# cgisky1980/Qwen3-TTS-Rust

Measured on AMD Instinct MI355X. Metric: audio_sec_per_s, higher is better.
Workload: dtype bf16

## Files before the change

qwen3-tts-rust_amd/csrc/q3_engine.h:

```cpp
#pragma once
#include <algorithm>
#include <cstddef>
#include <atomic>
#include <mutex>
#include <string>
#include <vector>

#include "../../include/q3tts.h"
#include "q3_kernels.h"

static_assert(sizeof(q3tts_request) == 80 && offsetof(q3tts_request, text_stream) == 12 && offsetof(q3tts_request, prompt) == 16 &&
              offsetof(q3tts_request, text_open) == 44 && offsetof(q3tts_request, seed) == 48 && offsetof(q3tts_request, prefix) == 72, "q3tts_request layout");

struct Q3Voc;
struct Q3Mel;
struct Q3Clone;

struct Q3Tfm {
    int L = 0, d = 0, Hq = 0, Hkv = 0, hd = 0, F = 0, nq = 0, nkv = 0, nqkv = 0, head_n = 0;
    std::vector<float*> attn_norm, ffn_norm, qn, kn;
    std::vector<uint4*> wqkv, wo, wgu, wd;
    float* out_norm = nullptr;
    uint4* head = nullptr;
    std::vector<uint16_t*> sqkv, so, sgu, sd; uint16_t* shead = nullptr; bool q8 = false;
// ... 49 lines not shown
    std::vector<float*> codec;
    const float** codec_dev = nullptr;
    std::vector<float*> pproj;
    float* proj_w = nullptr;
    float* proj_b = nullptr;
    float* qkv0 = nullptr;
    float* tts_pad = nullptr;
    float* marker_row = nullptr;
    int B = 0;
    std::vector<int> buckets; int cur_bucket = -1;
    std::vector<std::atomic<long long>> bucket_steps;
    std::atomic<long long> kvp_launches{0}, kvp_group_max{0};
    std::vector<int> row_of_slot, slot_of_row;
    Q3Slot* slots = nullptr;
    Q3Slot* slots_host = nullptr;
    int* codes = nullptr;
    float* rng = nullptr;
    Q3Lane lane;
    Q3Scratch sc_pre;
    Q3Rows pf;
    int *pf_pos = nullptr, *pf_slot = nullptr;
    int* pf_seg = nullptr;
    Q3PromptRow* prow_dev = nullptr; int prow_cap = 0;
    float* spk_dev = nullptr; int* refcodes_dev = nullptr;
    float temperature = 0.7f; int top_k = 40; float top_p = 0.9f; int has_seed = 0; uint64_t seed = 0;
    int max_steps = 512;
    float p_temperature = 0.0f; int p_top_k = 0; float p_top_p = 1.0f; float rep_penalty = 1.0f;
    int pred_force = 0, pred_variant = 0;
    int streams_open = 0;
    int* ts_ids = nullptr; int* ts_cnt = nullptr; int2* ts_cur = nullptr;
    std::vector<char> ts_slot; int ts_variant = 0, ts_used = 0;
    float* prng = nullptr;
    uint32_t* seen = nullptr; int seen_words = 0;
    hipEvent_t ev0 = nullptr, ev1 = nullptr, ev2 = nullptr, ev3 = nullptr;
    std::vector<hipEvent_t> fin_ev;
    q3tts_timings tm{};
    Q3Voc* voc = nullptr;
    Q3Mel* mel = nullptr;
    Q3Clone* clone = nullptr;
    int probe = 0, probe_kind = 0;
    std::vector<hipEvent_t> probe_ev;
    int probe_i = 0;
    double probe_ms = 0, probe_empty_ms = 0; long long probe_cnt = 0, probe_empty_cnt = 0, row_steps = 0;
    int dev_pcm_on = 0; float* dev_pcm = nullptr; int dev_pcm_n = 0; size_t dev_pcm_stride = 0;
    int out_rate = 0; Q3Resamp rs_out{}; std::vector<Q3Resamp> rs_cache;
    float* rs_stage = nullptr; size_t rs_stage_stride = 0, rs_stage_cap = 0;
    double hp_launch = 0, hp_sync = 0;
    float *park_logits = nullptr, *park_x = nullptr;
    float* first_chunk_host = nullptr;
    std::atomic<q3tts_session*> session{nullptr};
    std::mutex err_mu;
};

struct q3tts_prefix {
    q3tts_engine* e = nullptr;
    int P = 0, np = 0;
    uint16_t *k = nullptr, *v = nullptr;
    std::atomic<int> state{1};
    bool released = false; int qrefs = 0;
};
size_t q3_prefix_store_bytes(const q3tts_engine* e, int np);

int q3_set_err(q3tts_engine* e, int code, const std::string& msg);
int q3_refuse_in_session(q3tts_engine* e);
#define Q3_NOT_IN_SESSION(e) do { if ((e) && (e)->session.load()) return q3_refuse_in_session(e); } while (0)
#define Q3_HIP(e, call)                                                                                         \
    do {                                                                                                        \
// ... 52 lines not shown
int q3_launch_gemm(q3tts_engine* e, const Q3Tfm& t, const Q3BGemm& g, hipStream_t s, hipEvent_t* probe = nullptr, int kind = -1);

void q3_rope_tables(int n_pos, int hd, float theta, const int* sections, std::vector<float>& cs, std::vector<float>& sn);

void q3_stdrng_f32(uint64_t seed, int n, float* out);

void q3_mel_destroy(q3tts_engine* e);
int q3_mel_run(q3tts_engine* e, const float* audio, int64_t n_samples, int32_t* n_frames, float** out_dev);
void q3_clone_destroy(q3tts_engine* e);
int q3_voc_create(q3tts_engine* e);
void q3_voc_destroy(q3tts_engine* e);
int q3_voc_reset(q3tts_engine* e, int slot);
int q3_voc_decode(q3tts_engine* e, int slot, int f0, int nf, int is_last, hipStream_t s);
int q3_voc_decode_batch(q3tts_engine* e, const int* slots, const int* real, int ns, int nf, hipStream_t s, int beside_decoder);
void q3_voc_mark_last(q3tts_engine* e, int slot);
float* q3_voc_pcm(q3tts_engine* e, int slot);
int q3_voc_samples(q3tts_engine* e, int slot);
int q3_voc_samples_per_frame(const q3tts_engine* e);
size_t q3_voc_pcm_stride(const q3tts_engine* e);

int q3_resample_get(q3tts_engine* e, int rate_in, int rate_out, Q3Resamp* out);
int q3_resample_slot(q3tts_engine* e, int b, long long first_out, int count, int n_valid, bool is_final, hipStream_t s);

enum { BOS_TOKEN = 151672, EOS_TOKEN = 151673 };

int q3_plan_rows(q3tts_engine* e, const std::vector<int>& live);
int q3_admit_many(q3tts_engine* e, const int* slots, const q3tts_request* const* reqs, int count, int* rc);
struct Q3AdmItem {
    int slot; const q3tts_request* r;
    q3tts_prefix* keep; int keep_rows;
    const q3tts_prompt_desc* voice; const float* embd; int n_tok;
};
int q3_admit_items(q3tts_engine* e, const Q3AdmItem* items, int count, int* rc);
int q3_run_chunk(q3tts_engine* e, int CH);
int q3_clone_audio_encode_run(q3tts_engine* e, const float* audio, int64_t n_samples, int64_t* codes, int32_t cap_frames, int32_t* n_frames);
int q3_clone_speaker_encode_run(q3tts_engine* e, const float* audio, int64_t n_samples, float* spk_emb);
int q3_resample_run(q3tts_engine* e, const float* in, int64_t n_in, int32_t rate_in, int32_t rate_out, float* out, int64_t cap, int64_t* n_out);
int q3_text_rows_set(q3tts_engine* e, int b, const int32_t* T, int from, int n, int n_frames);
int q3_park_rows(q3tts_engine* e, int b, bool save);
void q3_text_trailing(const q3tts_request* r, std::vector<int32_t>& T);
int q3_pred_force_variant(q3tts_engine* e, int force);
int q3_voc_dispatch(q3tts_engine* e, const char* live, const char* want, int* voc_frames, bool more, bool* first);
double q3_now_ms();
```

qwen3-tts-rust_amd/csrc/q3_engine.hip:

```cpp
#include "q3_engine.h"
#include "q3_gguf.h"

#include <chrono>
#include <cmath>
#include <cstdio>
#include <cstdlib>
#include <cstring>

static thread_local std::string g_err;

int q3_set_err(q3tts_engine* e, int code, const std::string& msg) {
    if (e) { std::lock_guard<std::mutex> lk(e->err_mu); e->err = msg; }
    g_err = msg;
    return code;
}
extern "C" const char* q3tts_last_error(const q3tts_engine* e) {
    if (!e) return g_err.c_str();
    if (!e->session.load()) return e->err.c_str();
    static thread_local std::string copy;
    std::lock_guard<std::mutex> lk(const_cast<q3tts_engine*>(e)->err_mu);
    copy = e->err;
    return copy.c_str();
}
int q3_refuse_in_session(q3tts_engine* e) {
// ... 175 lines not shown
                              std::to_string(mm.t_head_dim) + ", ratio " + std::to_string(R) + ", n_ctx = " + std::to_string(cfg->n_ctx));
    }
    int ndev = 0;
    if (hipGetDeviceCount(&ndev) != hipSuccess || ndev <= 0)
        return q3_set_err(nullptr, Q3TTS_ERR_DEVICE, "no HIP device: libq3tts has no CPU fallback");
    if (cfg->device < 0 || cfg->device >= ndev) return q3_set_err(nullptr, Q3TTS_ERR_INVALID, "device ordinal out of range");
    q3tts_engine* e = new q3tts_engine();
    e->cfg = *cfg; e->cfg.weights_path = nullptr;
    e->max_steps = cfg->max_steps_cap < 512 ? cfg->max_steps_cap : 512;
    auto fail = [&](int rc) { std::string m = e->err; q3tts_engine_destroy(e); g_err = m; return rc; };
#define TRYC(x) do { int rc__ = (x); if (rc__ != Q3TTS_OK) return fail(rc__); } while (0)
#define HIPC(call) do { hipError_t er__ = (call); if (er__ != hipSuccess) { q3_set_err(e, Q3TTS_ERR_DEVICE, std::string(#call) + ": " + hipGetErrorString(er__)); return fail(Q3TTS_ERR_DEVICE); } } while (0)
    HIPC(hipSetDevice(cfg->device));
    {
        size_t free_b = 0, total_b = 0;
        HIPC(hipMemGetInfo(&free_b, &total_b));
        const unsigned long long need = engine_footprint(*cfg);
        if (need > (unsigned long long)free_b) {
            q3_set_err(e, Q3TTS_ERR_OOM, "engine needs at least " + std::to_string(need) + " bytes of device memory for max_batch = " + std::to_string(cfg->max_batch) +
                       ", n_ctx = " + std::to_string(cfg->n_ctx) + (cfg->kv_q8_0 ? " (Q8_0 cache)" : "") + "; the device has " + std::to_string((unsigned long long)free_b) +
                       (cfg->kv_q8_0 ? " bytes free (fewer slots or a smaller n_ctx)" : " bytes free (fewer slots, a smaller n_ctx, or kv_q8_0 = 1: the cache in 0.53 of the bytes)"));
            return fail(Q3TTS_ERR_OOM);
        }
    }
    q3_bgemm_prepare();
    if (cfg->talker_q8_0 == 2 || cfg->predictor_q8_0 == 2) q3_bgemm8_prepare();
    HIPC(hipStreamCreateWithFlags(&e->stream, hipStreamNonBlocking));
    if (getenv("Q3TTS_VOC_SERIAL") && atoi(getenv("Q3TTS_VOC_SERIAL"))) e->vstream = e->stream;
    else if (getenv("Q3TTS_VOC_CUMASK")) {
        uint32_t w = (uint32_t)strtoul(getenv("Q3TTS_VOC_CUMASK"), nullptr, 16), mask[8];
        for (auto& x : mask) x = w;
        HIPC(hipExtStreamCreateWithCUMask(&e->vstream, 8, mask));
    } else HIPC(hipStreamCreateWithFlags(&e->vstream, hipStreamNonBlocking));
    HIPC(hipEventCreate(&e->ev0)); HIPC(hipEventCreate(&e->ev1)); HIPC(hipEventCreate(&e->ev2)); HIPC(hipEventCreate(&e->ev3));
    e->fin_ev.resize(cfg->max_batch, nullptr);
    for (auto& ev : e->fin_ev) HIPC(hipEventCreateWithFlags(&ev, hipEventDisableTiming));
    const q3tts_model_config& m = e->cfg.model;
    const int B = cfg->max_batch;
    e->B = B;
    hipStream_t s = e->stream;
    const std::string wdir = cfg->weights_path ? cfg->weights_path : "";
    Q3Gguf gt, gp;
    std::string er;
    if (!wdir.empty() && (gt.open(wdir + "/qwen3_tts_talker.gguf", er) || gp.open(wdir + "/qwen3_tts_predictor.gguf", er))) { q3_set_err(e, Q3TTS_ERR_INVALID, er); return fail(Q3TTS_ERR_INVALID); }
    TRYC(q3_tfm_init(e, e->T, {.grp = Q3G_TALKER, .L = m.t_n_layer, .d = m.t_d_model, .Hq = m.t_n_head, .Hkv = m.t_n_kv_head, .hd = m.t_head_dim, .F = m.t_d_ffn,
                               .head_n = m.t_vocab, .theta = m.t_rope_theta, .sections = m.t_mrope_sections, .n_ctx = cfg->n_ctx, .n_slots = B, .kv8 = cfg->kv_q8_0},
                     wdir.empty() ? nullptr : &gt, "qwen3_tts_talker.gguf", cfg->talker_q8_0));
    TRYC(q3_tfm_init(e, e->P, {.grp = Q3G_PRED, .L = m.p_n_layer, .d = m.p_d_model, .Hq = m.p_n_head, .Hkv = m.p_n_kv_head, .hd = m.p_head_dim, .F = m.p_d_ffn,
                               .head_n = (m.n_codebooks - 1) * m.codebook_size, .theta = m.p_rope_theta, .sections = nullptr, .n_ctx = 64, .n_slots = B, .kv8 = 0},
                     wdir.empty() ? nullptr : &gp, "qwen3_tts_predictor.gguf", cfg->predictor_q8_0));
    TRYC(q3_assets_init(e, wdir));
    TRYC(q3_pred_table_init(e));
    TRYC(q3_dalloc(e, &e->slots, (size_t)B));
    HIPC(hipHostMalloc((void**)&e->slots_host, sizeof(Q3Slot) * 2 * B, hipHostMallocDefault));
    memset(e->slots_host, 0, sizeof(Q3Slot) * 2 * B);
    TRYC(q3_dalloc(e, &e->codes, (size_t)B * cfg->max_steps_cap * m.n_codebooks)); TRYC(q3_dalloc(e, &e->rng, (size_t)B * cfg->max_steps_cap));
    TRYC(q3_dalloc(e, &e->prng, (size_t)B * cfg->max_steps_cap * (m.n_codebooks - 1)));
    e->seen_words = (m.sample_limit + 31) / 32;
    TRYC(q3_dalloc(e, &e->seen, (size_t)B * e->seen_words));
    TRYC(q3_dalloc(e, &e->ts_ids, (size_t)B * cfg->max_steps_cap)); TRYC(q3_dalloc(e, &e->ts_cnt, (size_t)B)); TRYC(q3_dalloc(e, &e->ts_cur, (size_t)B));
    TRYC(q3_dalloc(e, &e->park_logits, (size_t)B * m.t_vocab)); TRYC(q3_dalloc(e, &e->park_x, (size_t)B * m.t_d_model));
    e->ts_slot.assign(B, 0);
    {
        const int nb = B;
        const int nqkv_max = std::max(e->T.nqkv, e->P.nqkv), nq_max = std::max(e->T.nq, e->P.nq), F_max = std::max(e->T.F, e->P.F);
        Q3Lane& L = e->lane;
        L.nb = nb;
// ... 43 lines not shown
    return Q3TTS_OK;
}

extern "C" void q3tts_engine_destroy(q3tts_engine* e) {
    if (!e) return;
    if (q3tts_session* ss = e->session.load()) q3tts_session_close(ss);
    hipSetDevice(e->cfg.device);
    if (e->stream) hipStreamSynchronize(e->stream);
    if (e->vstream) hipStreamSynchronize(e->vstream);
    if (e->voc) q3_voc_destroy(e);
    q3_mel_destroy(e);
    q3_clone_destroy(e);
    if (e->first_chunk_host) hipHostFree(e->first_chunk_host);
    {
        Q3Lane& L = e->lane;
        if (L.stream) hipStreamSynchronize(L.stream);
        for (auto ge : L.execs) if (ge) hipGraphExecDestroy(ge);
        for (auto gr : L.graphs) if (gr) hipGraphDestroy(gr);
        for (auto ge : L.execs_s) if (ge) hipGraphExecDestroy(ge);
        for (auto gr : L.graphs_s) if (gr) hipGraphDestroy(gr);
        for (int v = 0; v < 2; ++v) {
            for (auto ge : L.execs_t[v]) if (ge) hipGraphExecDestroy(ge);
            for (auto gr : L.graphs_t[v]) if (gr) hipGraphDestroy(gr);
        }
        if (L.ev_begin) hipEventDestroy(L.ev_begin); if (L.ev_end) hipEventDestroy(L.ev_end);
        if (L.stream) hipStreamDestroy(L.stream);
    }
    for (void* p : e->allocs) hipFree(p);
    hipFree(e->dev_pcm);
    hipFree(e->rs_stage);
    if (e->slots_host) hipHostFree(e->slots_host);
    for (auto ev : e->fin_ev) if (ev) hipEventDestroy(ev);
    for (auto ev : e->probe_ev) if (ev) hipEventDestroy(ev);
    if (e->ev0) hipEventDestroy(e->ev0); if (e->ev1) hipEventDestroy(e->ev1); if (e->ev2) hipEventDestroy(e->ev2); if (e->ev3) hipEventDestroy(e->ev3);
    if (e->stream) hipStreamDestroy(e->stream);
    if (e->vstream && e->vstream != e->stream) hipStreamDestroy(e->vstream);
    delete e;
}

extern "C" int q3tts_set_sampler(q3tts_engine* e, float temperature, int32_t top_k, float top_p, int32_t has_seed, uint64_t seed) {
    if (!e) return q3_set_err(nullptr, Q3TTS_ERR_INVALID, "null engine");
    Q3_NOT_IN_SESSION(e);
    e->temperature = temperature; e->top_k = top_k; e->top_p = top_p; e->has_seed = has_seed; e->seed = seed;
    return Q3TTS_OK;
}
static int refuse_busy(q3tts_engine* e) {
    if (e->streams_open > 0) return q3_set_err(e, Q3TTS_ERR_STATE, "a stream is open on this engine (q3tts_stream_end first)");
    return Q3TTS_OK;
}
static int set_pred_variant(q3tts_engine* e, int variant) {
    if (variant && e->cfg.model.codebook_size > Q3_SAMP_MAX) return q3_set_err(e, Q3TTS_ERR_INVALID, "the Predictor sampler needs codebook_size <= 4096");
    if (!variant) { e->pred_variant = 0; return Q3TTS_OK; }
    Q3_HIP(e, hipSetDevice(e->cfg.device));
    if (q3_pred_next_prepare() != 0) return q3_set_err(e, Q3TTS_ERR_DEVICE, "the Predictor sampler's kernel: the device refused its LDS size (hipFuncSetAttribute)");
    e->pred_variant = variant;
    Q3Lane& L = e->lane;
    if (!L.execs.empty() && L.execs_s.empty()) {
        Q3_HIP(e, hipStreamSynchronize(e->stream));
        const int rc = q3_capture_frames(e, L.graphs_s, L.execs_s);
        if (rc != Q3TTS_OK) {
            for (auto ge : L.execs_s) if (ge) hipGraphExecDestroy(ge);
            for (auto gr : L.graphs_s) if (gr) hipGraphDestroy(gr);
            L.execs_s.clear(); L.graphs_s.clear(); e->pred_variant = 0;
            return rc;
        }
    }
    return Q3TTS_OK;
// ... 141 lines not shown
    return Q3TTS_OK;
}

static int plan_rows(q3tts_engine* e, const std::vector<int>& live_in) {
    Q3Lane& L = e->lane;
    const int B = e->B;
    std::vector<int> live(live_in);
    std::sort(live.begin(), live.end());
    int bi = 0;
    while (bi + 1 < (int)e->buckets.size() && e->buckets[bi] < (int)live.size()) ++bi;
    bool ok = bi == e->cur_bucket;
    if (ok) for (int b : live) if (e->row_of_slot[b] >= e->buckets[bi]) { ok = false; break; }
    if (ok) return Q3TTS_OK;
    std::vector<int> slot_of_row(B, -1), perm(B), used(B, 0);
    int r = 0;
    for (int b : live) { slot_of_row[r++] = b; used[b] = 1; }
    for (int b = 0; b < B && r < B; ++b) if (!used[b]) slot_of_row[r++] = b;
    for (r = 0; r < B; ++r) perm[r] = e->row_of_slot[slot_of_row[r]];
    hipStream_t s = e->stream;
    Q3_HIP(e, hipMemcpyAsync(L.perm, perm.data(), (size_t)B * 4, hipMemcpyHostToDevice, s));
    Q3_HIP(e, hipMemcpyAsync(L.slot_id, slot_of_row.data(), (size_t)B * 4, hipMemcpyHostToDevice, s));
    q3_launch_gather_rows(L.logits_tmp, L.logits, L.perm, B, e->cfg.model.t_vocab, s);
    Q3_HIP(e, hipMemcpyAsync(L.logits, L.logits_tmp, (size_t)B * e->cfg.model.t_vocab * 4, hipMemcpyDeviceToDevice, s));
    q3_launch_gather_rows(L.logits_tmp, L.T.x, L.perm, B, e->cfg.model.t_d_model, s);
    Q3_HIP(e, hipMemcpyAsync(L.T.x, L.logits_tmp, (size_t)B * e->cfg.model.t_d_model * 4, hipMemcpyDeviceToDevice, s));
    Q3_HIP(e, hipStreamSynchronize(s));
    for (r = 0; r < B; ++r) e->row_of_slot[slot_of_row[r]] = r;
    e->slot_of_row = slot_of_row;
    e->cur_bucket = bi;
    return Q3TTS_OK;
}

static double now_ms();
static int run_chunk(q3tts_engine* e, int CH, float* dev_ms) {
    hipStream_t s = e->stream;
    Q3Lane& L = e->lane;
    const double hp0 = now_ms();
    Q3_HIP(e, hipEventRecord(e->ev1, s));
    Q3_HIP(e, hipStreamWaitEvent(L.stream, e->ev1, 0));
    Q3_HIP(e, hipEventRecord(L.ev_begin, L.stream));
    e->probe_i = 0;
    if (e->probe) { hipEventRecord(e->probe_ev[8], L.stream); hipEventRecord(e->probe_ev[9], L.stream); }
    bool ts = false;
    for (char f : e->ts_slot) ts |= f != 0;
    e->ts_variant = ts ? 1 : 0;
    const std::vector<hipGraphExec_t>& execs = ts ? L.execs_t[e->pred_variant ? 1 : 0] : e->pred_variant ? L.execs_s : L.execs;
    for (int i = 0; i < CH; ++i) {
        if (!execs.empty() && !e->probe) { Q3_HIP(e, hipGraphLaunch(execs[e->cur_bucket], L.stream)); }
        else {
            if (q3_record_frame(e, L, L.stream, e->buckets[e->cur_bucket])) return q3_set_err(e, Q3TTS_ERR_INVALID, "frame step: a kernel launch was refused for this model shape");
            Q3_HIP(e, hipGetLastError());
        }
    }
    e->row_steps += (long long)CH * e->buckets[e->cur_bucket];
    e->bucket_steps[e->cur_bucket].fetch_add(CH, std::memory_order_relaxed);
    Q3_HIP(e, hipEventRecord(L.ev_end, L.stream));
    Q3_HIP(e, hipStreamWaitEvent(s, L.ev_end, 0));
    Q3_HIP(e, hipEventRecord(e->ev3, s));
    Q3_HIP(e, hipMemcpyAsync(e->slots_host, e->slots, sizeof(Q3Slot) * e->B, hipMemcpyDeviceToHost, s));
    const double hp1 = now_ms();
    Q3_HIP(e, hipStreamSynchronize(s));
    e->hp_launch += hp1 - hp0; e->hp_sync += now_ms() - hp1;
    if (dev_ms) { *dev_ms = 0.0f; hipEventElapsedTime(dev_ms, L.ev_begin, L.ev_end); }
    for (int i = 0; i + 1 < e->probe_i; i += 2) {
        float ms = 0.0f;
        if (hipEventElapsedTime(&ms, e->probe_ev[i], e->probe_ev[i + 1]) == hipSuccess) { e->probe_ms += ms; ++e->probe_cnt; }
    }
    if (e->probe) {
        float ms = 0.0f;
        if (hipEventElapsedTime(&ms, e->probe_ev[8], e->probe_ev[9]) == hipSuccess) { e->probe_empty_ms += ms; ++e->probe_empty_cnt; }
    }
    return Q3TTS_OK;
}

static uint64_t wall_seed() {
    return (uint64_t)std::chrono::duration_cast<std::chrono::nanoseconds>(std::chrono::system_clock::now().time_since_epoch()).count();
}

struct Adm { int b; const q3tts_request* r; int n, row0, max_steps, P; q3tts_prefix* keep; int keep_rows; };

void q3_text_trailing(const q3tts_request* r, std::vector<int32_t>& T) {
    T.clear();
    const q3tts_prompt_desc* p = r->prompt;
    for (int i = 1; p && i < p->n_text; ++i) T.push_back((int32_t)p->text_ids[i]);
    if (!(r->text_open == 1)) T.push_back(EOS_TOKEN);
}
int q3_text_rows_set(q3tts_engine* e, int b, const int32_t* T, int from, int n, int n_frames) {
    const int cap = e->cfg.max_steps_cap, c = std::min(std::max(n, 0), cap);
    hipStream_t s = e->stream;
    from = std::max(from, 0);
    if (from < c) Q3_HIP(e, hipMemcpyAsync(e->ts_ids + (size_t)b * cap + from, T + from, (size_t)(c - from) * 4, hipMemcpyHostToDevice, s));
    const int2 cur = n_frames >= 0 && n_frames < c ? make_int2(1, T[n_frames]) : make_int2(0, 0);
    Q3_HIP(e, hipMemcpyAsync(e->ts_cnt + b, &c, 4, hipMemcpyHostToDevice, s));
    Q3_HIP(e, hipMemcpyAsync(e->ts_cur + b, &cur, sizeof(cur), hipMemcpyHostToDevice, s));
    Q3_HIP(e, hipStreamSynchronize(s));
    return Q3TTS_OK;
}
int q3_park_rows(q3tts_engine* e, int b, bool save) {
    const q3tts_model_config& m = e->cfg.model;
    Q3Lane& L = e->lane;
    const size_t row = (size_t)e->row_of_slot[b], nl = (size_t)m.t_vocab, nx = (size_t)m.t_d_model;
    float *lg = L.logits + row * nl, *x = L.T.x + row * nx, *plg = e->park_logits + (size_t)b * nl, *px = e->park_x + (size_t)b * nx;
    Q3_HIP(e, hipMemcpyAsync(save ? plg : lg, save ? lg : plg, nl * 4, hipMemcpyDeviceToDevice, e->stream));
    Q3_HIP(e, hipMemcpyAsync(save ? px : x, save ? x : px, nx * 4, hipMemcpyDeviceToDevice, e->stream));
    return Q3TTS_OK;
// ... 252 lines not shown
    for (int i = 0; i < n; ++i) pos[i] = i;
    uint16_t *kc = t.kc, *vc = t.vc, *kd = t.kd, *vd = t.vd; const size_t ls = t.layer_stride; const int nc = t.n_ctx;
    t.kc = x->k; t.vc = x->v; t.layer_stride = (size_t)t.Hkv * x->np * t.hd; t.n_ctx = x->np;
    if (t.kv8) { t.kd = (uint16_t*)((int8_t*)x->k + per); t.vd = (uint16_t*)((int8_t*)x->v + per); }
    const int rl = prefill_layers(e, pos, zero, {0, n, 0, 0}, n, n, nullptr);
    t.kc = kc; t.vc = vc; t.kd = kd; t.vd = vd; t.layer_stride = ls; t.n_ctx = nc;
    if (rl < 0) return fail(Q3TTS_ERR_DEVICE, std::string(e->err));
    if (rl) return fail(Q3TTS_ERR_INVALID, "prefix: a kernel launch was refused for this model shape");
    hipError_t er = hipGetLastError();
    if (er == hipSuccess) er = hipStreamSynchronize(s);
    if (er != hipSuccess) return fail(Q3TTS_ERR_DEVICE, hipGetErrorString(er));
    *out = x;
    return Q3TTS_OK;
}
extern "C" int32_t q3tts_prefix_rows(const q3tts_prefix* x) { return x && x->state.load(std::memory_order_acquire) == 1 ? x->P : 0; }
extern "C" int32_t q3tts_prefix_state(const q3tts_prefix* x) { return x ? x->state.load(std::memory_order_acquire) : Q3TTS_ERR_INVALID; }
extern "C" int q3tts_prefix_destroy(q3tts_prefix* x) {
    if (!x) return Q3TTS_OK;
    q3tts_engine* e = x->e;
    Q3_NOT_IN_SESSION(e);
    hipSetDevice(e->cfg.device);
    hipStreamSynchronize(e->stream);
    hipFree(x->k); hipFree(x->v);
    delete x;
    return Q3TTS_OK;
}

static double now_ms() {
    return std::chrono::duration<double, std::milli>(std::chrono::steady_clock::now().time_since_epoch()).count();
}

struct SlotRun { int req = -1; double t_first = 0; };

int q3_voc_dispatch(q3tts_engine* e, const char* live, const char* want, int* voc_frames, bool more, bool* first) {
    const int B = e->B;
    hipStream_t vs = e->vstream;
    bool waited = false;
    *first = false;
    auto ensure_wait = [&]() -> int { if (!waited) { Q3_HIP(e, hipStreamWaitEvent(vs, e->ev3, 0)); waited = true; } return Q3TTS_OK; };
    std::vector<int> list(B), real(B);
    for (;;) {
        int ns = 0;
        for (int b = 0; b < B; ++b) {
            if (!live[b] || !want[b]) continue;
            const int pend = e->slots_host[b].n_frames - voc_frames[b];
            if (pend >= 4 || (pend > 0 && !e->slots_host[b].active)) { real[ns] = std::min(pend, 4); list[ns++] = b; }
        }
        if (!ns) break;
        TRY(ensure_wait());
        int still = 0;
        for (int b = 0; b < B; ++b) if (live[b] && e->slots_host[b].active) ++still;
        TRY(q3_voc_decode_batch(e, list.data(), real.data(), ns, 4, vs, (still > 0 || more) ? 1 : 0));
        for (int i = 0; i < ns; ++i) { if (voc_frames[list[i]] == 0) *first = true; voc_frames[list[i]] += real[i]; }
    }
    for (int b = 0; b < B; ++b)
        if (live[b] && !e->slots_host[b].active && (e->cfg.vocoder_flush_tail || e->slots_host[b].n_frames % 4 != 0)) q3_voc_mark_last(e, b);
    return Q3TTS_OK;
}

#include <mutex>
namespace {
struct PinHdr { size_t cap; size_t magic; };
std::mutex g_pin_mu;
std::vector<PinHdr*> g_pin_pool;
size_t g_pin_bytes = 0;
float* pin_alloc(size_t bytes) {
    {
        std::lock_guard<std::mutex> lk(g_pin_mu);
        for (size_t i = 0; i < g_pin_pool.size(); ++i)
            if (g_pin_pool[i]->cap >= bytes && g_pin_pool[i]->cap <= 2 * bytes + 4096) {
                PinHdr* h = g_pin_pool[i];
                g_pin_pool[i] = g_pin_pool.back(); g_pin_pool.pop_back(); g_pin_bytes -= h->cap;
                return (float*)((char*)h + 64);
            }
    }
    void* p = nullptr;
    const size_t cap = (bytes + 65535) & ~(size_t)65535;
    if (hipHostMalloc(&p, cap + 64, hipHostMallocDefault) != hipSuccess) return nullptr;
    PinHdr* h = (PinHdr*)p; h->cap = cap; h->magic = 0x5133505043ull;
    return (float*)((char*)p + 64);
}
void pin_free(float* q) {
    if (!q) return;
    PinHdr* h = (PinHdr*)((char*)q - 64);
    if (h->magic != 0x5133505043ull) return;
    std::lock_guard<std::mutex> lk(g_pin_mu);
    if (g_pin_pool.size() < 256 && g_pin_bytes + h->cap <= ((size_t)1 << 30)) { g_pin_pool.push_back(h); g_pin_bytes += h->cap; return; }
    hipHostFree(h);
}
}

static int finalize(q3tts_engine* e, int b, const q3tts_request* r, q3tts_result* o, const SlotRun& sr, double t0, bool defer = false,
                    hipEvent_t fin_ev = nullptr, int ri = -1) {
    const int ncb = e->cfg.model.n_codebooks;
    const Q3Slot& st = e->slots_host[b];
    o->n_frames = st.n_frames; o->hit_eos = st.hit_eos;
    o->codes = (int32_t*)malloc(sizeof(int32_t) * (size_t)std::max(1, st.n_frames * ncb));
    if (!o->codes) return q3_set_err(e, Q3TTS_ERR_OOM, "malloc");
    if (st.n_frames > 0)
        Q3_HIP(e, hipMemcpyAsync(o->codes, e->codes + (size_t)b * e->cfg.max_steps_cap * ncb, sizeof(int32_t) * (size_t)st.n_frames * ncb,
                                 hipMemcpyDeviceToHost, e->stream));
    o->sample_rate = e->out_rate && e->voc ? e->out_rate : e->cfg.vocoder.sample_rate;
    if (r->want_pcm && e->voc && e->dev_pcm && ri >= 0 && ri < e->dev_pcm_n) {
        const int ns = q3_voc_samples(e, b);
        if (ns > 0) Q3_HIP(e, hipMemcpyAsync(e->dev_pcm + (size_t)ri * e->dev_pcm_stride, q3_voc_pcm(e, b), sizeof(float) * (size_t)ns, hipMemcpyDeviceToDevice, e->vstream));
    }
    if (r->want_pcm == 2 && e->voc) {
        o->n_samples = q3_voc_samples(e, b);
        if (defer) Q3_HIP(e, hipEventRecord(fin_ev, e->vstream));
        else Q3_HIP(e, hipStreamSynchronize(e->vstream));
    } else if (r->want_pcm && e->voc) {
        int ns = q3_voc_samples(e, b);
        const float* from = q3_voc_pcm(e, b);
        if (e->out_rate) {
            const int no = (int)q3_resample_N(ns, e->rs_out.L, e->rs_out.M);
            TRY(q3_resample_slot(e, b, 0, no, ns, true, e->vstream));
            ns = no; from = e->rs_stage + (size_t)b * e->rs_stage_stride;
        }
        o->n_samples = ns;
        o->pcm = pin_alloc(sizeof(float) * (size_t)std::max(1, ns));
        if (!o->pcm) return q3_set_err(e, Q3TTS_ERR_OOM, "hipHostMalloc");
        if (ns > 0) Q3_HIP(e, hipMemcpyAsync(o->pcm, from, sizeof(float) * (size_t)ns, hipMemcpyDeviceToHost, e->vstream));
        if (defer) Q3_HIP(e, hipEventRecord(fin_ev, e->vstream));
        else Q3_HIP(e, hipStreamSynchronize(e->vstream));
    } else if (defer) {
        Q3_HIP(e, hipEventRecord(fin_ev, e->vstream));
    }
    Q3_HIP(e, hipStreamSynchronize(e->stream));
    o->first_chunk_ms = sr.t_first > 0 ? (float)(sr.t_first - t0) : 0.0f;
    o->total_ms = (float)(now_ms() - t0);
    o->status = defer ? Q3TTS_ERR_STATE : Q3TTS_OK;
    return Q3TTS_OK;
}

static int complete_result(q3tts_engine* e, q3tts_result* o, hipEvent_t fin_ev, double t0) {
    Q3_HIP(e, hipEventSynchronize(fin_ev));
    o->total_ms = (float)(now_ms() - t0);
    o->status = Q3TTS_OK;
    return Q3TTS_OK;
}

extern "C" int q3tts_generate_batch(q3tts_engine* e, const q3tts_request* reqs, int32_t n, q3tts_result* outs) {
    if (!e || !reqs || !outs || n <= 0) return q3_set_err(e, Q3TTS_ERR_INVALID, "null/empty argument");
    Q3_NOT_IN_SESSION(e);
    Q3_HIP(e, hipSetDevice(e->cfg.device));
    for (int i = 0; i < n; ++i) { memset(&outs[i], 0, sizeof(outs[i])); outs[i].status = Q3TTS_ERR_STATE; }
    for (int i = 0; i < n; ++i) {
        if (reqs[i].want_pcm && !e->voc) return q3_set_err(e, Q3TTS_ERR_STATE, "want_pcm on an engine created with with_vocoder = 0");
        if (reqs[i].want_pcm == 2 && !e->dev_pcm_on) return q3_set_err(e, Q3TTS_ERR_STATE, "want_pcm = 2 (device only) needs q3tts_set_device_pcm(engine, 1)");
        if (reqs[i].text_open == 1) return q3_set_err(e, Q3TTS_ERR_INVALID, "text_open = 1 is for sessions (q3tts_session_append_text): this call takes closed text and never waits");
    }
    std::fill(e->ts_slot.begin(), e->ts_slot.end(), 0);
    if (e->dev_pcm_on && e->voc) {
        const size_t stride = (size_t)e->cfg.max_steps_cap * q3_voc_samples_per_frame(e);
        if (e->dev_pcm_n < n || e->dev_pcm_stride != stride) {
            if (e->dev_pcm) { Q3_HIP(e, hipStreamSynchronize(e->vstream)); hipFree(e->dev_pcm); e->dev_pcm = nullptr; e->dev_pcm_n = 0; }
            void* p = nullptr;
            if (hipMalloc(&p, (size_t)n * stride * sizeof(float)) != hipSuccess) return q3_set_err(e, Q3TTS_ERR_OOM, "hipMalloc (device PCM)");
            e->dev_pcm = (float*)p; e->dev_pcm_n = n; e->dev_pcm_stride = stride;
        }
    }
    const int B = e->B, CH = 4;
    const int spf = e->voc ? q3_voc_samples_per_frame(e) : 0;
    std::vector<SlotRun> run(B);
    std::vector<int> voc_frames(B, 0);
    std::vector<char> live(B, 0), want(B, 0);
    const double t0 = now_ms();
    std::vector<int> pending(B, -1);
    auto drain = [&](int b) -> int {
        if (pending[b] >= 0) { TRY(complete_result(e, &outs[pending[b]], e->fin_ev[b], t0)); pending[b] = -1; }
        return Q3TTS_OK;
    };
    int next = 0, done = 0;
    double dec_ms = 0, pre_ms = 0, voc_ms = 0;
    static const bool host_prof = [] { const char* ev = getenv("Q3TTS_HOST_PROF"); return ev && atoi(ev); }();
    double hp_admit = 0, hp_chunk = 0, hp_voc = 0, hp_fin = 0, hp_tail = 0, hp_t = now_ms();
    auto hp_lap = [&](double& acc) { if (host_prof) { const double t = now_ms(); acc += t - hp_t; hp_t = t; } };
    long long steps = 0, ctx_tokens = 0, live_slot_steps = 0;
    e->probe_ms = 0; e->probe_cnt = 0; e->row_steps = 0; e->probe_empty_ms = 0; e->probe_empty_cnt = 0;
    hipStream_t s = e->stream;
    while (done < n) {
        bool admitted = false;
        {
            std::vector<int> as, ai; std::vector<const q3tts_request*> ar;
            for (int b = 0; b < B && next < n; ++b)
                if (run[b].req < 0) { TRY(drain(b)); as.push_back(b); ar.push_back(&reqs[next]); ai.push_back(next++); }
            {
                std::vector<int> live(as);
                for (int b = 0; b < B; ++b) if (run[b].req >= 0) live.push_back(b);
                TRY(plan_rows(e, live));
            }
            if (!as.empty()) {
                Q3_HIP(e, hipEventRecord(e->ev0, s));
                admitted = true;
                std::vector<int> rcs(as.size());
                TRY(admit_many(e, as.data(), ar.data(), (int)as.size(), rcs.data()));
                for (size_t i = 0; i < as.size(); ++i) {
                    if (rcs[i] != Q3TTS_OK) { outs[ai[i]].status = rcs[i]; ++done; }
                    else { run[as[i]] = SlotRun{}; run[as[i]].req = ai[i]; voc_frames[as[i]] = 0; }
                }
            }
        }
        if (admitted) { Q3_HIP(e, hipEventRecord(e->ev2, s)); }
        hp_lap(hp_admit);
        bool any = false;
        for (int b = 0; b < B; ++b) if (run[b].req >= 0) any = true;
        if (!any) break;
        float ms = 0;
        TRY(run_chunk(e, CH, &ms));
        hp_lap(hp_chunk);
        dec_ms += ms; steps += CH;
        if (admitted) { hipEventElapsedTime(&ms, e->ev0, e->ev2); pre_ms += ms; }
        for (int b = 0; b < B; ++b) if (run[b].req >= 0) { ctx_tokens += (long long)e->slots_host[b].cur_pos * CH; live_slot_steps += CH; }
        if (e->voc) {
            const double tv0 = now_ms();
            hipStream_t vs = e->vstream;
            for (int b = 0; b < B; ++b) { live[b] = run[b].req >= 0; want[b] = live[b] && reqs[run[b].req].want_pcm; }
            bool first = false;
            TRY(q3_voc_dispatch(e, live.data(), want.data(), voc_frames.data(), next < n, &first));
            if (first) {
                for (int b = 0; b < B; ++b)
                    if (run[b].req >= 0 && run[b].t_first == 0 && voc_frames[b] > 0) {
                        const int nsmp = std::min(voc_frames[b], 4) * spf;
                        Q3_HIP(e, hipMemcpyAsync(e->first_chunk_host, q3_voc_pcm(e, b), sizeof(float) * (size_t)nsmp, hipMemcpyDeviceToHost, vs));
                    }
                Q3_HIP(e, hipStreamSynchronize(vs));
                const double tn = now_ms();
                for (int b = 0; b < B; ++b) if (run[b].req >= 0 && run[b].t_first == 0 && voc_frames[b] > 0) run[b].t_first = tn;
            }
            voc_ms += now_ms() - tv0;
        }
        hp_lap(hp_voc);
        for (int j = 0; j < B; ++j)
            if (pending[j] >= 0 && hipEventQuery(e->fin_ev[j]) == hipSuccess) TRY(drain(j));
        for (int b = 0; b < B; ++b) {
            if (run[b].req < 0 || e->slots_host[b].active) continue;
            for (int j = 0; j < B; ++j)
                if (pending[j] >= 0 && hipEventQuery(e->fin_ev[j]) == hipSuccess) TRY(drain(j));
            TRY(finalize(e, b, &reqs[run[b].req], &outs[run[b].req], run[b], t0, true, e->fin_ev[b], run[b].req));
            pending[b] = run[b].req;
            run[b].req = -1; ++done;
            e->ts_slot[b] = 0;
        }
        hp_lap(hp_fin);
    }
    for (int b = 0; b < B; ++b) TRY(drain(b));
    hp_lap(hp_tail);
    if (host_prof) {
        fprintf(stderr, "q3tts_generate_batch host wall (ms): admit + plan %.1f | chunks (launch + wait) %.1f = launch %.1f + wait %.1f, device events %.1f over %lld steps | vocoder issue %.1f | finalize %.1f | tail (last results) %.1f | total %.1f\n",
                hp_admit, hp_chunk, e->hp_launch, e->hp_sync, dec_ms, steps, hp_voc, hp_fin, hp_tail, now_ms() - t0);
        e->hp_launch = e->hp_sync = 0;
    }
    e->tm.prefill_ms = (float)pre_ms; e->tm.decode_ms = (float)dec_ms; e->tm.vocoder_ms = (float)voc_ms;
    e->tm.total_ms = (float)(now_ms() - t0); e->tm.frame_steps = steps; e->tm.frame_step_ms = steps ? (float)(dec_ms / steps) : 0.0f;
    {
        const q3tts_model_config& m = e->cfg.model;
        const long long wt = (long long)e->T.weight_bytes;
        const double bpw_p = e->P.q8 ? 1.0625 : 2.0;
        const long long wp_layers = (long long)e->P.weight_bytes - (long long)(bpw_p * (double)((size_t)e->P.head_n * m.p_d_model));
        const long long head1 = (long long)(bpw_p * (double)((size_t)m.codebook_size * m.p_d_model)), pj = 2ll * m.p_d_model * m.d_embed;
        const long long kv_per_tok = 2ll * m.t_n_layer * 2 * m.t_n_kv_head * m.t_head_dim;
        long long fixed = wt + (m.n_codebooks - 1) * (wp_layers + head1) + pj;
        e->tm.mean_live_slots = steps ? (float)((double)live_slot_steps / (double)steps) : 0.0f;
        long long gathered = 0;
        if (q3_pred_table_on(e)) {
            fixed -= (long long)(m.n_codebooks - 2) * (long long)(bpw_p * (double)((size_t)e->P.nqkv * m.p_d_model));
            gathered = (long long)((double)(m.n_codebooks - 2) * (double)e->tm.mean_live_slots * (double)e->P.nqkv * 4.0);
        }
        e->tm.algo_bytes_per_step = fixed + gathered + (steps ? kv_per_tok * (ctx_tokens / steps) : 0);
        e->tm.algo_flops_per_step = (long long)((double)fixed * (double)e->tm.mean_live_slots);
        e->tm.mean_rows = steps ? (float)((double)e->row_steps / (double)steps) : 0.0f;
        e->tm.mean_ctx_tokens = steps ? (float)((double)ctx_tokens / (double)steps) : 0.0f;
        e->tm.probe_kernel_ms = e->probe_cnt ? (float)(e->probe_ms / (double)e->probe_cnt) : 0.0f;
        e->tm.probe_count = e->probe_cnt;
        e->tm.probe_empty_ms = e->probe_empty_cnt ? (float)(e->probe_empty_ms / (double)e->probe_empty_cnt) : 0.0f;
    }
    return Q3TTS_OK;
}

int q3_plan_rows(q3tts_engine* e, const std::vector<int>& live) { return plan_rows(e, live); }
int q3_admit_many(q3tts_engine* e, const int* slots, const q3tts_request* const* reqs, int count, int* rc) { return admit_many(e, slots, reqs, count, rc); }
int q3_admit_items(q3tts_engine* e, const Q3AdmItem* items, int count, int* rc) { return admit_items(e, items, count, rc); }
int q3_run_chunk(q3tts_engine* e, int CH) { return run_chunk(e, CH, nullptr); }
double q3_now_ms() { return now_ms(); }

extern "C" int q3tts_generate(q3tts_engine* e, const q3tts_request* req, q3tts_result* out) {
    int rc = q3tts_generate_batch(e, req, 1, out);
    if (rc != Q3TTS_OK) return rc;
    return out->status;
}

extern "C" void q3tts_result_free(q3tts_result* r) {
    if (!r) return;
    free(r->codes);
    pin_free(r->pcm);
    r->codes = nullptr; r->pcm = nullptr;
}

extern "C" int q3tts_get_timings(const q3tts_engine* e, q3tts_timings* out) {
    if (!e || !out) return Q3TTS_ERR_INVALID;
    *out = e->tm;
    return Q3TTS_OK;
}

struct q3tts_stream {
    q3tts_engine* e; q3tts_request req; int voc_frames = 0; bool finished = false; bool final_sent = false;
    std::vector<float> chunk; double t0 = 0, t_first = 0;
    long long delivered = 0;
};

static int stream_emit(q3tts_stream* st, int before, int after, bool fin, const float** chunk, int32_t* n_samples) {
    q3tts_engine* e = st->e;
    hipStream_t s = e->stream;
    const float* from = q3_voc_pcm(e, 0) + before;
    int c = after - before;
// ... 50 lines not shown
            TRY(q3_voc_decode(e, 0, st->voc_frames, nf, last, s));
            st->voc_frames += nf;
            const int after = q3_voc_samples(e, 0);
            const bool fin = st->finished && st->voc_frames >= sl.n_frames;
            TRY(stream_emit(st, before, after, fin, chunk, n_samples));
            if (st->t_first == 0) st->t_first = now_ms();
            if (fin) { *is_final = 1; st->final_sent = true; }
            (void)spf;
            return Q3TTS_OK;
        }
        if (st->finished) {
            const int before = q3_voc_samples(e, 0);
            if (e->cfg.vocoder_flush_tail) q3_voc_mark_last(e, 0);
            const int after = q3_voc_samples(e, 0);
            if (after > before || (e->out_rate && q3_resample_N(after, e->rs_out.L, e->rs_out.M) > st->delivered))
                TRY(stream_emit(st, before, after, true, chunk, n_samples));
            *is_final = 1; st->final_sent = true; return Q3TTS_OK;
        }
    }
}

extern "C" int q3tts_stream_end(q3tts_stream* st, q3tts_result* out) {
    if (!st) return Q3TTS_ERR_INVALID;
    q3tts_engine* e = st->e;
    int rc = Q3TTS_OK;
    Q3Slot* stage = e->slots_host + e->B;
    memset(stage, 0, sizeof(Q3Slot));
    hipMemcpyAsync(e->slots_host, e->slots, sizeof(Q3Slot), hipMemcpyDeviceToHost, e->stream);
    hipStreamSynchronize(e->stream);
    if (out) {
        memset(out, 0, sizeof(*out));
        SlotRun sr; sr.t_first = st->t_first;
        q3tts_request r = st->req; r.want_pcm = 1;
        rc = finalize(e, 0, &r, out, sr, st->t0);
    }
    hipMemcpyAsync(e->slots, stage, sizeof(Q3Slot), hipMemcpyHostToDevice, e->stream);
    hipStreamSynchronize(e->stream);
    --e->streams_open;
    e->ts_slot[0] = 0;
    delete st;
    return rc;
}
```

qwen3-tts-rust_amd/csrc/q3_session.hip:

```cpp
#include "q3_engine.h"

#include <chrono>
#include <condition_variable>
#include <cstring>
#include <deque>
#include <map>
#include <memory>
#include <thread>

namespace {

#define TRY(x) do { int rc__ = (x); if (rc__ != Q3TTS_OK) return rc__; } while (0)

constexpr int kRing = Q3TTS_SESSION_RING_DEPTH;
constexpr int kStopping = 1;

struct SReq {
    uint64_t id = 0;
    q3tts_request r{};
    q3tts_prompt_desc desc{};
    std::vector<float> embd, spk;
    std::vector<uint32_t> text, instr, ref_text;
    std::vector<int32_t> ref_codes;
    int kind = 0, voice_rows = 0, n_tok = 0;
// ... 358 lines not shown
            q3_text_trailing(&sl.req->r, T0);
            sl.t_up = sl.t_len = (int)T0.size(); sl.t_closed = !(sl.req->r.text_open == 1);
            tn[as[i]] = std::move(tn_adm[i]);
            TextNow& t = tn[as[i]];
            if (t.have) { sl.t_closed = t.closed; if ((int)t.T.size() > sl.t_len) sl.t_len = (int)t.T.size(); }
            nf[as[i]] = 0;
            if (!text_ready(sl, 0)) { TRY(park(s, as[i], e->slots_host[e->B + as[i]])); moved = true; }
        }
    }
    for (int b = 0; b < B; ++b) {
        SSlot& sl = s->slots[b];
        if (!sl.req || !sl.ts) continue;
        if (sl.parked) {
            if (!text_ready(sl, nf[b])) continue;
            TRY(resume(s, b)); moved = true;
        }
        if (sl.t_len > sl.t_up && (int)tn[b].T.size() >= sl.t_len) {
            TRY(q3_text_rows_set(e, b, tn[b].T.data(), sl.t_up, sl.t_len, nf[b]));
            sl.t_up = sl.t_len;
        }
    }
    if (moved) Q3_HIP(e, hipStreamSynchronize(e->stream));
    std::vector<char> run(B, 0);
    bool any = false;
    for (int b = 0; b < B; ++b) if (s->slots[b].req && !s->slots[b].parked) { run[b] = 1; any = true; }
    if (!any) {
        if (retired || made_prefix) Q3_HIP(e, hipStreamSynchronize(e->stream));
        if (!bt.evs.empty()) s->flight.push_back(std::move(bt));
        return Q3TTS_OK;
    }
    TRY(q3_run_chunk(e, 4));
    bool more, first = false;
    { std::lock_guard<std::mutex> lk(s->mu); more = !s->pending.empty(); }
    TRY(q3_voc_dispatch(e, run.data(), run.data(), s->voc_frames.data(), more, &first));
    const Q3Resamp* rs = e->out_rate ? &e->rs_out : nullptr;
    std::vector<Q3PcmEnt> ents; std::vector<int> ent_len; std::vector<char> ent_fin;
    int ne = 0;
    size_t tot = 0;
    std::vector<SEv> chunks;
    std::vector<int> fin;
    for (int b = 0; b < B; ++b) {
        if (!run[b]) continue;
        SSlot& sl = s->slots[b];
        const bool done = !e->slots_host[b].active;
        const int ns = q3_voc_samples(e, b);
        const int c = (rs ? (int)(done ? q3_resample_N(ns, rs->L, rs->M) : q3_resample_D(ns, rs->L, rs->M, rs->H)) : ns) - sl.delivered;
        if (c < 0 || tot + (size_t)std::max(c, 0) > s->ring_cap || ns > (int)q3_voc_pcm_stride(e))
            return q3_set_err(e, Q3TTS_ERR_STATE, "session: a chunk window exceeds the staging bound");
        if (c > 0 || done) {
            SEv v; v.id = sl.req->id; v.kind = Q3TTS_EV_CHUNK; v.n = c; v.is_final = done ? 1 : 0; v.off = tot;
            chunks.push_back(v);
        }
        if (c > 0) {
            ent_len.push_back(ns); ent_fin.push_back(done ? 1 : 0);
            ents.push_back(Q3PcmEnt{b, sl.delivered, c, 0, (long long)tot}); ++ne;
            tot += (size_t)c; sl.delivered += c;
        }
        if (done) fin.push_back(b);
    }
    if (ne > 0) {
        const int k = s->ring_next;
        const int rc = take_ring(s, k);
        if (rc) return rc;
        for (int g0 = 0; g0 < ne; g0 += Q3_PCM_MAX_ENT) {
            const int n = std::min(ne - g0, (int)Q3_PCM_MAX_ENT);
            Q3PcmPack pk{}; Q3PcmSrc src{};
            int mx = 0;
// ... 402 lines not shown
```

Before: 682.6.

## Issue next decode chunk before host vocoder/finalize work to overlap host and device

Splits run_chunk into issue and wait halves. After a chunk completes and no new admissions are needed, the batch loop snapshots slot state and launches the next decode chunk before doing vocoder dispatch and finalize, so that host work runs beside the GPU. Finalize copies codes on the vocoder stream after waiting on a double-buffered chunk-end event instead of synchronizing the decode stream. This adds snapshot copies and event ping-ponging, and it risks ordering bugs on slot state.

Result: no change. 683.3, median of 2 (+0.1%).

```diff
diff --git a/qwen3-tts-rust_amd/csrc/q3_engine.h b/qwen3-tts-rust_amd/csrc/q3_engine.h
--- a/qwen3-tts-rust_amd/csrc/q3_engine.h
+++ b/qwen3-tts-rust_amd/csrc/q3_engine.h
@@ -105,7 +105,8 @@
     std::vector<char> ts_slot; int ts_variant = 0, ts_used = 0;
     float* prng = nullptr;
     uint32_t* seen = nullptr; int seen_words = 0;
-    hipEvent_t ev0 = nullptr, ev1 = nullptr, ev2 = nullptr, ev3 = nullptr;
+    hipEvent_t ev0 = nullptr, ev1 = nullptr, ev2 = nullptr;
+    hipEvent_t ev_ce[2] = {nullptr, nullptr}, ev3 = nullptr; int ce_next = 0, ce_issued = 0;
     std::vector<hipEvent_t> fin_ev;
     q3tts_timings tm{};
     Q3Voc* voc = nullptr;
@@ -224,6 +225,8 @@
     const q3tts_prompt_desc* voice; const float* embd; int n_tok;
 };
 int q3_admit_items(q3tts_engine* e, const Q3AdmItem* items, int count, int* rc);
+int q3_issue_chunk(q3tts_engine* e, int CH);
+int q3_wait_chunk(q3tts_engine* e, float* dev_ms);
 int q3_run_chunk(q3tts_engine* e, int CH);
 int q3_clone_audio_encode_run(q3tts_engine* e, const float* audio, int64_t n_samples, int64_t* codes, int32_t cap_frames, int32_t* n_frames);
 int q3_clone_speaker_encode_run(q3tts_engine* e, const float* audio, int64_t n_samples, float* spk_emb);
@@ -232,5 +235,5 @@
 int q3_park_rows(q3tts_engine* e, int b, bool save);
 void q3_text_trailing(const q3tts_request* r, std::vector<int32_t>& T);
 int q3_pred_force_variant(q3tts_engine* e, int force);
-int q3_voc_dispatch(q3tts_engine* e, const char* live, const char* want, int* voc_frames, bool more, bool* first);
+int q3_voc_dispatch(q3tts_engine* e, const Q3Slot* mir, const char* live, const char* want, int* voc_frames, bool more, bool* first);
 double q3_now_ms();
diff --git a/qwen3-tts-rust_amd/csrc/q3_engine.hip b/qwen3-tts-rust_amd/csrc/q3_engine.hip
--- a/qwen3-tts-rust_amd/csrc/q3_engine.hip
+++ b/qwen3-tts-rust_amd/csrc/q3_engine.hip
@@ -231,7 +231,8 @@
         for (auto& x : mask) x = w;
         HIPC(hipExtStreamCreateWithCUMask(&e->vstream, 8, mask));
     } else HIPC(hipStreamCreateWithFlags(&e->vstream, hipStreamNonBlocking));
-    HIPC(hipEventCreate(&e->ev0)); HIPC(hipEventCreate(&e->ev1)); HIPC(hipEventCreate(&e->ev2)); HIPC(hipEventCreate(&e->ev3));
+    HIPC(hipEventCreate(&e->ev0)); HIPC(hipEventCreate(&e->ev1)); HIPC(hipEventCreate(&e->ev2));
+    HIPC(hipEventCreate(&e->ev_ce[0])); HIPC(hipEventCreate(&e->ev_ce[1])); e->ev3 = e->ev_ce[0];
     e->fin_ev.resize(cfg->max_batch, nullptr);
     for (auto& ev : e->fin_ev) HIPC(hipEventCreateWithFlags(&ev, hipEventDisableTiming));
     const q3tts_model_config& m = e->cfg.model;
@@ -341,7 +342,8 @@
     if (e->slots_host) hipHostFree(e->slots_host);
     for (auto ev : e->fin_ev) if (ev) hipEventDestroy(ev);
     for (auto ev : e->probe_ev) if (ev) hipEventDestroy(ev);
-    if (e->ev0) hipEventDestroy(e->ev0); if (e->ev1) hipEventDestroy(e->ev1); if (e->ev2) hipEventDestroy(e->ev2); if (e->ev3) hipEventDestroy(e->ev3);
+    if (e->ev0) hipEventDestroy(e->ev0); if (e->ev1) hipEventDestroy(e->ev1); if (e->ev2) hipEventDestroy(e->ev2);
+    for (hipEvent_t ev : e->ev_ce) if (ev) hipEventDestroy(ev);
     if (e->stream) hipStreamDestroy(e->stream);
     if (e->vstream && e->vstream != e->stream) hipStreamDestroy(e->vstream);
     delete e;
@@ -549,7 +551,7 @@
 }
 
 static double now_ms();
-static int run_chunk(q3tts_engine* e, int CH, float* dev_ms) {
+static int issue_chunk(q3tts_engine* e, int CH) {
     hipStream_t s = e->stream;
     Q3Lane& L = e->lane;
     const double hp0 = now_ms();
@@ -573,11 +575,18 @@
     e->bucket_steps[e->cur_bucket].fetch_add(CH, std::memory_order_relaxed);
     Q3_HIP(e, hipEventRecord(L.ev_end, L.stream));
     Q3_HIP(e, hipStreamWaitEvent(s, L.ev_end, 0));
-    Q3_HIP(e, hipEventRecord(e->ev3, s));
+    e->ce_issued = e->ce_next; e->ce_next ^= 1;
+    Q3_HIP(e, hipEventRecord(e->ev_ce[e->ce_issued], s));
     Q3_HIP(e, hipMemcpyAsync(e->slots_host, e->slots, sizeof(Q3Slot) * e->B, hipMemcpyDeviceToHost, s));
+    e->hp_launch += now_ms() - hp0;
+    return Q3TTS_OK;
+}
+static int wait_chunk(q3tts_engine* e, float* dev_ms) {
+    Q3Lane& L = e->lane;
     const double hp1 = now_ms();
-    Q3_HIP(e, hipStreamSynchronize(s));
-    e->hp_launch += hp1 - hp0; e->hp_sync += now_ms() - hp1;
+    Q3_HIP(e, hipStreamSynchronize(e->stream));
+    e->ev3 = e->ev_ce[e->ce_issued];
+    e->hp_sync += now_ms() - hp1;
     if (dev_ms) { *dev_ms = 0.0f; hipEventElapsedTime(dev_ms, L.ev_begin, L.ev_end); }
     for (int i = 0; i + 1 < e->probe_i; i += 2) {
         float ms = 0.0f;
@@ -588,6 +597,10 @@
         if (hipEventElapsedTime(&ms, e->probe_ev[8], e->probe_ev[9]) == hipSuccess) { e->probe_empty_ms += ms; ++e->probe_empty_cnt; }
     }
     return Q3TTS_OK;
+}
+static int run_chunk(q3tts_engine* e, int CH, float* dev_ms) {
+    TRY(issue_chunk(e, CH));
+    return wait_chunk(e, dev_ms);
 }
 
 static uint64_t wall_seed() {
@@ -906,7 +919,7 @@
 
 struct SlotRun { int req = -1; double t_first = 0; };
 
-int q3_voc_dispatch(q3tts_engine* e, const char* live, const char* want, int* voc_frames, bool more, bool* first) {
+int q3_voc_dispatch(q3tts_engine* e, const Q3Slot* mir, const char* live, const char* want, int* voc_frames, bool more, bool* first) {
     const int B = e->B;
     hipStream_t vs = e->vstream;
     bool waited = false;
@@ -917,18 +930,18 @@
         int ns = 0;
         for (int b = 0; b < B; ++b) {
             if (!live[b] || !want[b]) continue;
-            const int pend = e->slots_host[b].n_frames - voc_frames[b];
-            if (pend >= 4 || (pend > 0 && !e->slots_host[b].active)) { real[ns] = std::min(pend, 4); list[ns++] = b; }
+            const int pend = mir[b].n_frames - voc_frames[b];
+            if (pend >= 4 || (pend > 0 && !mir[b].active)) { real[ns] = std::min(pend, 4); list[ns++] = b; }
         }
         if (!ns) break;
         TRY(ensure_wait());
         int still = 0;
-        for (int b = 0; b < B; ++b) if (live[b] && e->slots_host[b].active) ++still;
+        for (int b = 0; b < B; ++b) if (live[b] && mir[b].active) ++still;
         TRY(q3_voc_decode_batch(e, list.data(), real.data(), ns, 4, vs, (still > 0 || more) ? 1 : 0));
         for (int i = 0; i < ns; ++i) { if (voc_frames[list[i]] == 0) *first = true; voc_frames[list[i]] += real[i]; }
     }
     for (int b = 0; b < B; ++b)
-        if (live[b] && !e->slots_host[b].active && (e->cfg.vocoder_flush_tail || e->slots_host[b].n_frames % 4 != 0)) q3_voc_mark_last(e, b);
+        if (live[b] && !mir[b].active && (e->cfg.vocoder_flush_tail || mir[b].n_frames % 4 != 0)) q3_voc_mark_last(e, b);
     return Q3TTS_OK;
 }
 
@@ -964,16 +977,18 @@
 }
 }
 
-static int finalize(q3tts_engine* e, int b, const q3tts_request* r, q3tts_result* o, const SlotRun& sr, double t0, bool defer = false,
-                    hipEvent_t fin_ev = nullptr, int ri = -1) {
+static int finalize(q3tts_engine* e, int b, const Q3Slot& st, const q3tts_request* r, q3tts_result* o, const SlotRun& sr, double t0, bool defer = false,
+                    hipEvent_t fin_ev = nullptr, int ri = -1, hipEvent_t chunk_ev = nullptr) {
     const int ncb = e->cfg.model.n_codebooks;
-    const Q3Slot& st = e->slots_host[b];
+    const bool ahead = defer && chunk_ev;
+    hipStream_t cs = ahead ? e->vstream : e->stream;
     o->n_frames = st.n_frames; o->hit_eos = st.hit_eos;
     o->codes = (int32_t*)malloc(sizeof(int32_t) * (size_t)std::max(1, st.n_frames * ncb));
     if (!o->codes) return q3_set_err(e, Q3TTS_ERR_OOM, "malloc");
+    if (ahead) Q3_HIP(e, hipStreamWaitEvent(cs, chunk_ev, 0));
     if (st.n_frames > 0)
         Q3_HIP(e, hipMemcpyAsync(o->codes, e->codes + (size_t)b * e->cfg.max_steps_cap * ncb, sizeof(int32_t) * (size_t)st.n_frames * ncb,
-                                 hipMemcpyDeviceToHost, e->stream));
+                                 hipMemcpyDeviceToHost, cs));
     o->sample_rate = e->out_rate && e->voc ? e->out_rate : e->cfg.vocoder.sample_rate;
     if (r->want_pcm && e->voc && e->dev_pcm && ri >= 0 && ri < e->dev_pcm_n) {
         const int ns = q3_voc_samples(e, b);
@@ -1000,7 +1015,7 @@
     } else if (defer) {
         Q3_HIP(e, hipEventRecord(fin_ev, e->vstream));
     }
-    Q3_HIP(e, hipStreamSynchronize(e->stream));
+    if (!ahead) Q3_HIP(e, hipStreamSynchronize(e->stream));
     o->first_chunk_ms = sr.t_first > 0 ? (float)(sr.t_first - t0) : 0.0f;
     o->total_ms = (float)(now_ms() - t0);
     o->status = defer ? Q3TTS_ERR_STATE : Q3TTS_OK;
@@ -1053,9 +1068,19 @@
     long long steps = 0, ctx_tokens = 0, live_slot_steps = 0;
     e->probe_ms = 0; e->probe_cnt = 0; e->row_steps = 0; e->probe_empty_ms = 0; e->probe_empty_cnt = 0;
     hipStream_t s = e->stream;
+    static const bool order_new = [] { const char* ev = getenv("Q3TTS_CHUNK_ORDER"); return !ev || atoi(ev) != 0; }();
+    std::vector<Q3Slot> snap(B);
+    bool issued = false;
+    double hp_empty = 0, hp_over = 0, hp_wait_end = 0, hp_issue_end = 0;
+    auto issue = [&]() -> int {
+        if (host_prof && hp_wait_end > 0) hp_empty += now_ms() - hp_wait_end;
+        TRY(issue_chunk(e, CH));
+        if (host_prof) hp_issue_end = now_ms();
+        return Q3TTS_OK;
+    };
     while (done < n) {
         bool admitted = false;
-        {
+        if (!issued) {
             std::vector<int> as, ai; std::vector<const q3tts_request*> ar;
             for (int b = 0; b < B && next < n; ++b)
                 if (run[b].req < 0) { TRY(drain(b)); as.push_back(b); ar.push_back(&reqs[next]); ai.push_back(next++); }
@@ -1075,23 +1100,43 @@
                 }
             }
         }
-        if (admitted) { Q3_HIP(e, hipEventRecord(e->ev2, s)); }
-        hp_lap(hp_admit);
-        bool any = false;
-        for (int b = 0; b < B; ++b) if (run[b].req >= 0) any = true;
-        if (!any) break;
+        if (!issued) {
+            if (admitted) { Q3_HIP(e, hipEventRecord(e->ev2, s)); }
+            hp_lap(hp_admit);
+            bool any = false;
+            for (int b = 0; b < B; ++b) if (run[b].req >= 0) any = true;
+            if (!any) break;
+            TRY(issue());
+        }
+        issued = false;
         float ms = 0;
-        TRY(run_chunk(e, CH, &ms));
+        if (host_prof) hp_over += now_ms() - hp_issue_end;
+        TRY(wait_chunk(e, &ms));
+        if (host_prof) hp_wait_end = now_ms();
         hp_lap(hp_chunk);
         dec_ms += ms; steps += CH;
         if (admitted) { hipEventElapsedTime(&ms, e->ev0, e->ev2); pre_ms += ms; }
-        for (int b = 0; b < B; ++b) if (run[b].req >= 0) { ctx_tokens += (long long)e->slots_host[b].cur_pos * CH; live_slot_steps += CH; }
+        memcpy(snap.data(), e->slots_host, sizeof(Q3Slot) * (size_t)B);
+        for (int b = 0; b < B; ++b) if (run[b].req >= 0) { ctx_tokens += (long long)snap[b].cur_pos * CH; live_slot_steps += CH; }
+        if (order_new) {
+            std::vector<int> lv;
+            for (int b = 0; b < B; ++b) if (run[b].req >= 0 && snap[b].active) lv.push_back(b);
+            const bool refill = next < n && (int)lv.size() < B;
+            if (!refill && !lv.empty()) {
+                for (int b = 0; b < B; ++b) if (run[b].req >= 0 && !snap[b].active) e->ts_slot[b] = 0;
+                TRY(plan_rows(e, lv));
+                hp_lap(hp_admit);
+                TRY(issue());
+                hp_lap(hp_chunk);
+                issued = true;
+            }
+        }
         if (e->voc) {
             const double tv0 = now_ms();
             hipStream_t vs = e->vstream;
             for (int b = 0; b < B; ++b) { live[b] = run[b].req >= 0; want[b] = live[b] && reqs[run[b].req].want_pcm; }
             bool first = false;
-            TRY(q3_voc_dispatch(e, live.data(), want.data(), voc_frames.data(), next < n, &first));
+            TRY(q3_voc_dispatch(e, snap.data(), live.data(), want.data(), voc_frames.data(), next < n, &first));
             if (first) {
                 for (int b = 0; b < B; ++b)
                     if (run[b].req >= 0 && run[b].t_first == 0 && voc_frames[b] > 0) {
@@ -1108,10 +1153,10 @@
         for (int j = 0; j < B; ++j)
             if (pending[j] >= 0 && hipEventQuery(e->fin_ev[j]) == hipSuccess) TRY(drain(j));
         for (int b = 0; b < B; ++b) {
-            if (run[b].req < 0 || e->slots_host[b].active) continue;
+            if (run[b].req < 0 || snap[b].active) continue;
             for (int j = 0; j < B; ++j)
                 if (pending[j] >= 0 && hipEventQuery(e->fin_ev[j]) == hipSuccess) TRY(drain(j));
-            TRY(finalize(e, b, &reqs[run[b].req], &outs[run[b].req], run[b], t0, true, e->fin_ev[b], run[b].req));
+            TRY(finalize(e, b, snap[b], &reqs[run[b].req], &outs[run[b].req], run[b], t0, true, e->fin_ev[b], run[b].req, issued ? e->ev3 : nullptr));
             pending[b] = run[b].req;
             run[b].req = -1; ++done;
             e->ts_slot[b] = 0;
@@ -1121,8 +1166,8 @@
     for (int b = 0; b < B; ++b) TRY(drain(b));
     hp_lap(hp_tail);
     if (host_prof) {
-        fprintf(stderr, "q3tts_generate_batch host wall (ms): admit + plan %.1f | chunks (launch + wait) %.1f = launch %.1f + wait %.1f, device events %.1f over %lld steps | vocoder issue %.1f | finalize %.1f | tail (last results) %.1f | total %.1f\n",
-                hp_admit, hp_chunk, e->hp_launch, e->hp_sync, dec_ms, steps, hp_voc, hp_fin, hp_tail, now_ms() - t0);
+        fprintf(stderr, "q3tts_generate_batch host wall (ms): admit + plan %.1f | chunks (launch + wait) %.1f = launch %.1f + wait %.1f, device events %.1f over %lld steps | vocoder issue %.1f | finalize %.1f | tail (last results) %.1f | total %.1f | between chunks, decode stream empty %.1f | host work beside a running chunk %.1f (chunk order %d)\n",
+                hp_admit, hp_chunk, e->hp_launch, e->hp_sync, dec_ms, steps, hp_voc, hp_fin, hp_tail, now_ms() - t0, hp_empty, hp_over, order_new ? 1 : 0);
         e->hp_launch = e->hp_sync = 0;
     }
     e->tm.prefill_ms = (float)pre_ms; e->tm.decode_ms = (float)dec_ms; e->tm.vocoder_ms = (float)voc_ms;
@@ -1155,6 +1200,8 @@
 int q3_plan_rows(q3tts_engine* e, const std::vector<int>& live) { return plan_rows(e, live); }
 int q3_admit_many(q3tts_engine* e, const int* slots, const q3tts_request* const* reqs, int count, int* rc) { return admit_many(e, slots, reqs, count, rc); }
 int q3_admit_items(q3tts_engine* e, const Q3AdmItem* items, int count, int* rc) { return admit_items(e, items, count, rc); }
+int q3_issue_chunk(q3tts_engine* e, int CH) { return issue_chunk(e, CH); }
+int q3_wait_chunk(q3tts_engine* e, float* dev_ms) { return wait_chunk(e, dev_ms); }
 int q3_run_chunk(q3tts_engine* e, int CH) { return run_chunk(e, CH, nullptr); }
 double q3_now_ms() { return now_ms(); }
 
@@ -1271,7 +1318,7 @@
         memset(out, 0, sizeof(*out));
         SlotRun sr; sr.t_first = st->t_first;
         q3tts_request r = st->req; r.want_pcm = 1;
-        rc = finalize(e, 0, &r, out, sr, st->t0);
+        rc = finalize(e, 0, e->slots_host[0], &r, out, sr, st->t0);
     }
     hipMemcpyAsync(e->slots, stage, sizeof(Q3Slot), hipMemcpyHostToDevice, e->stream);
     hipStreamSynchronize(e->stream);
diff --git a/qwen3-tts-rust_amd/csrc/q3_session.hip b/qwen3-tts-rust_amd/csrc/q3_session.hip
--- a/qwen3-tts-rust_amd/csrc/q3_session.hip
+++ b/qwen3-tts-rust_amd/csrc/q3_session.hip
@@ -414,7 +414,7 @@
     TRY(q3_run_chunk(e, 4));
     bool more, first = false;
     { std::lock_guard<std::mutex> lk(s->mu); more = !s->pending.empty(); }
-    TRY(q3_voc_dispatch(e, run.data(), run.data(), s->voc_frames.data(), more, &first));
+    TRY(q3_voc_dispatch(e, e->slots_host, run.data(), run.data(), s->voc_frames.data(), more, &first));
     const Q3Resamp* rs = e->out_rate ? &e->rs_out : nullptr;
     std::vector<Q3PcmEnt> ents; std::vector<int> ent_len; std::vector<char> ent_fin;
     int ne = 0;
```
